# rhuangr/MARL-Maze

Measured on AMD Instinct MI355X. Metric: env-steps/sec (2-agent 10x10 maze) + PPO updates/sec, higher is better.
Workload: dtype f32; 1 GPU; PPO rollout+GAE+update over 65536 parallel 10x10 2-agent mazes per GPU (configs[2], the north-star workload: 65,536 parallel 10x10 mazes per GPU); mazes_per_gpu=65536, maze=10x10 (layout 19x19), horizon=16, global_batch=1048575, minibatch=209715, minibatch_steps_per_iter=25, parallelism=dp1, rollout=stream launches, gemm=x2, parity_mode=True

## Files before the change

include/marlmaze.h:

```cpp
#ifndef MARLMAZE_H
#define MARLMAZE_H

#include <stdint.h>

#ifdef __cplusplus
extern "C" {
#endif

#define MM_OBS_DIM 65
#define MM_MASK_DIM 6
#define MM_RNG_WORDS 625
#define MM_MAX_SIDE 41
#define MM_MAZES_PER_BLOCK 32

#define MM_E_ARG (-1)
#define MM_E_SIZE (-2)

#define MM_ST_GEN_FAIL 1u
#define MM_ST_BAD_MOVE 2u

typedef struct {
    int8_t x, y, dir, flags;
    int8_t lmx, lmy, olsx, olsy;
    int8_t minx, maxx, miny, maxy;
// ... 247 lines not shown
#define MM_PAR_HIST0 16
#define MM_PAR_HIST_BINS 16
int mm_par_init(uint64_t* totals, int32_t* counted, int n, void* stream);
int mm_par_accum(const uint8_t* done, const float* reward, const int32_t* ep_stats, const int32_t* par, int n,
                 int quota, int32_t* counted, uint64_t* totals, void* stream);

#define MM_ELOG_WORDS 16
#define MM_ELOG_LEN 0
#define MM_ELOG_SHORTEST 1
#define MM_ELOG_SOLVED 2
#define MM_ELOG_PAR 3
#define MM_ELOG_T_KEY 4
#define MM_ELOG_FETCHER 5
#define MM_ELOG_T_KNOW0 6
#define MM_ELOG_T_KNOW1 7
#define MM_ELOG_T_READY 8
#define MM_ELOG_CELLS0 9
#define MM_ELOG_CELLS1 10
#define MM_ELOG_CELLS_BOTH 11
#define MM_ELOG_OPEN 12
#define MM_ELOG_MARKS0 13
#define MM_ELOG_MARKS1 14
#define MM_ELOG_STAYS 15
long mm_elog_state_words(int layout_stride);
int mm_elog_init(int32_t* log, int32_t* counted, int32_t* state, int n, int quota, long state_words, void* stream);
int mm_elog_start(const mm_env_t* env, const uint8_t* select, int32_t* state, long state_words, void* stream);
int mm_elog_step(const mm_env_t* env, const int8_t* actions, const uint8_t* done, const float* reward,
                 const int32_t* ep_stats, const int32_t* par, int quota, int32_t* counted, int32_t* state,
                 long state_words, int32_t* log, void* stream);

int mm_critic_value(const float* x, int ldx, int K0, int M, int H0, int H1, const float* w0, const float* b0,
                    const float* w1, const float* b1, const float* w2, const float* b2, float* v, void* stream);

int mm_actor_front_ws_len(void);
int mm_actor_front_prep(const float* const* wproj, const float* const* bproj, const float* wq, const float* wk,
                        const float* wv, float* ws, void* stream);
int mm_actor_front_fwd(const float* ws, const float* x, int ldx, int B, int parity, float* h, void* stream);

#define MM_FRONT_FWD_ROW1 0
#define MM_FRONT_FWD_ROW2 1
#define MM_FRONT_FWD_MFMA 2
int mm_actor_front_fwd_ex(const float* ws, const float* x, int ldx, int B, int parity, float* h, int algo,
                          void* stream);

int mm_actor_front_grad_len(void);
int mm_actor_front_partial_len(void);
int mm_actor_front_bwd(const float* ws, const float* x, int ldx, int B, int parity, const float* dh, float* partial,
                       int grid, float* red, float* grad, void* stream);
#define MM_FRONT_BWD_MFMA 0
#define MM_FRONT_BWD_VALU 1
int mm_actor_front_bwd_ex(const float* ws, const float* x, int ldx, int B, int parity, const float* dh,
                          float* partial, int grid, float* red, float* grad, int algo, void* stream);
int mm_actor_front_bwd_grid(int B, int algo);
int mm_actor_front_bwd_to(const float* ws, const float* x, int ldx, int B, int parity, const float* dh,
                          float* partial, int grid, float* red, float* const* wproj_grad, float* const* bproj_grad,
                          float* wq_grad, float* wk_grad, float* wv_grad, int algo, void* stream);

#ifdef __cplusplus
}
#endif
#endif
```

marl-maze_amd/csrc/x3mlp.hip:

```cpp
#include <hip/hip_runtime.h>
#include <stdint.h>
#include <stdlib.h>

#include <algorithm>
#include <type_traits>

#include "marlmaze.h"
#include "policy_device.h"

namespace mm {
namespace x3 {

typedef __attribute__((ext_vector_type(8))) short bf16x8;
typedef __attribute__((ext_vector_type(4))) float f32x4;
typedef __attribute__((ext_vector_type(8))) _Float16 f16x8;

enum { P_X3 = MM_PREC_X3, P_F16 = MM_PREC_F16, P_X2 = MM_PREC_X2 };
template <int P>
struct Prec {
    static constexpr int kPlanes = P == P_X3 ? 3 : P == P_X2 ? 2 : 1;
    static constexpr int kBlk = 512 * kPlanes;
    static constexpr bool kScaled = P != P_X3;
};
constexpr float kX2Lo = 2048.f;
// ... 2369 lines not shown
                if (odd) bres_step<P, CT, RT, VW>(acc, accx, rawA, rawB, as, ks, K, kq, ctb, c0, ctn, ascale, sF, lane);
                if (half) {
#pragma unroll
                    for (int r = 0; r < RT; r++) bres_frag16<P, VW>(odd ? rawB[r] : rawA[r], ascale, a4[r]);
                }
            }
            if (half) {
                const uint2* bp = reinterpret_cast<const uint2*>(sT) + (size_t)(c0 * np) * 64 + lane;
#pragma unroll
                for (int c = 0; c < CT; c++) {
                    if (c < ctn) {
                        uint2 bb[3];
#pragma unroll
                        for (int q = 0; q < np; q++) bb[q] = bp[(c * np + q) * 64];
#pragma unroll
                        for (int r = 0; r < RT; r++) acc[r][c] = mma16<P>(a4[r], bb, acc[r][c], accx[r][c]);
                    }
                }
            }
#pragma unroll
            for (int r = 0; r < RT; r++)
#pragma unroll
                for (int c = 0; c < CT; c++) acc[r][c] = x2_combine<P>(acc[r][c], accx[r][c]);
#pragma unroll
            for (int r = 0; r < RT; r++)
                bres_epilogue<P, CT, EM>(acc[r], RT * u + r, t0 + c0, ctn, M, N, ep, crs, srs, sbias + 16 * c0, lane);
        }
        X3_STAMP(1 + t, 2, __builtin_amdgcn_s_memtime());
    }
    X3_STAMP(0, 3, __builtin_amdgcn_s_memtime());
    X3_STAMP(0, 5, __builtin_amdgcn_s_memrealtime());
}

}
}

using namespace mm::x3;

#ifdef X3_STAMPS
extern "C" int mm_x3_stamps_read(unsigned long long* out, long n) {
    const long cap = (long)(sizeof(g_x3_stamps) / sizeof(g_x3_stamps[0]));
    return hipMemcpyFromSymbol(out, HIP_SYMBOL(g_x3_stamps), (n < cap ? n : cap) * sizeof(unsigned long long), 0,
                               hipMemcpyDeviceToHost) == hipSuccess ? 0 : -1;
}
extern "C" int mm_trunk_stamps_read(unsigned long long* out, long n) {
    const long cap = (long)(sizeof(g_tr_stamps) / sizeof(g_tr_stamps[0]));
    return hipMemcpyFromSymbol(out, HIP_SYMBOL(g_tr_stamps), (n < cap ? n : cap) * sizeof(unsigned long long), 0,
                               hipMemcpyDeviceToHost) == hipSuccess ? 0 : -1;
}
extern "C" int mm_x3_stamps_clear() {
    static unsigned long long zero[256 * 16 * kWaves * 8];
    return hipMemcpyToSymbol(HIP_SYMBOL(g_x3_stamps), zero, sizeof(zero), 0, hipMemcpyHostToDevice) == hipSuccess
               ? 0 : -1;
}
#endif

extern "C" long mm_x3_tp_len(int R, int C) { return (long)(rup(R, kRowPad) / 16) * (rup(C, 32) / 32) * kBlk; }

extern "C" long mm_gemm_tp_len(int prec, int R, int C) {
    if (prec != MM_PREC_X3 && prec != MM_PREC_F16 && prec != MM_PREC_X2) return MM_E_ARG;
    return mm_x3_tp_len(R, C) / 3 * (prec == MM_PREC_X3 ? 3 : prec == MM_PREC_X2 ? 2 : 1);
}

extern "C" long mm_x3_mbits_len(int M) { return (long)(rup(M, kRowPad) / 16) * 64 * kMaskWords; }

extern "C" int mm_gemm_tp_pack(int prec, const float* X, int R, int C, int ld, int trans, uint16_t* tp,
// ... 826 lines not shown
}

extern "C" int mm_gemm_wgrad_partials_h(int prec, int flags, const float* dy, int lddy, float dscale, const void* x,
                                        int ldx, int M, int N, int K, float cscale, float* ws, void* stream) {
    if (M <= 0) return MM_E_ARG;
    return gemm_wgrad(prec, dy, lddy, dscale, static_cast<const float*>(x), ldx, M, N, K, cscale, ws, nullptr, stream,
                      flags);
}

extern "C" int mm_gemm_a16_ok(int M, int N, int K, int lda, int ldc) {
    BresPlan pl;
    int cfg = C_NARROW;
    return bres_enabled() && bres_plan(MM_PREC_F16, M, N, K, lda, ldc, true, pl, cfg) ? 1 : 0;
}

extern "C" int mm_gemm_x2p_ok(int M, int N, int K) {
    if (M <= 0 || N <= 0 || K <= 0 || N > 16 * kWgMaxT || (N & 3) || (K & 3)) return 0;
    if ((size_t)(M + 16) * std::max(N, K) * 4 >= ((size_t)1 << 31)) return 0;
    return wg_x2p_shape(wg_plan(MM_PREC_X2, M, N, K)) ? 1 : 0;
}

extern "C" int mm_gemm_wgrad_slices(int prec, int M, int N, int K) {
    if (M <= 0 || N <= 0 || K <= 0 || (prec != MM_PREC_X3 && prec != MM_PREC_F16 && prec != MM_PREC_X2))
        return MM_E_ARG;
    const WgPlan p = wg_plan(prec, M, N, K);
    return p.TPW ? p.nslices : MM_E_ARG;
}

extern "C" int mm_gemm_wgrad_partials(int prec, const float* dy, int lddy, float dscale, const float* x, int ldx, int M,
                                      int N, int K, float cscale, float* ws, void* stream) {
    if (M <= 0) return MM_E_ARG;
    return gemm_wgrad(prec, dy, lddy, dscale, x, ldx, M, N, K, cscale, ws, nullptr, stream);
}
```

marl-maze_amd/marlmaze/PPO.py:

```python
import math
import os
import random
import warnings

import numpy as np
import torch

from . import _lib, networks, ops, rollout, update, x3
from .dist import DP
from .networks import Actor, Critic

MODEL_PATH = "PPO.pth"
CRITIC_STREAM = os.environ.get("MARLMAZE_CRITIC_STREAM", "on")
CRITIC_STREAM_MAX_SAMPLES = int(os.environ.get("MARLMAZE_CRITIC_STREAM_MAX", "65536"))


def _ppo_loss_fwd(heads, mk, a8, old_logp, adv, clip):
    L = _lib.lib()
    M = old_logp.shape[0]
    old_logp, adv = old_logp.contiguous(), adv.contiguous()
    coef = torch.empty(M, dtype=torch.float32, device=heads.device)
    part = torch.empty(L.mm_ppo_loss_partials(M), dtype=torch.float32, device=heads.device)
    _lib.check(L.mm_ppo_loss(_lib.ptr(heads), _lib.ptr(mk), _lib.ptr(a8), _lib.ptr(old_logp), _lib.ptr(adv), M,
                             float(clip), _lib.ptr(coef), _lib.ptr(part), _lib.stream_ptr()), "mm_ppo_loss")
# ... 138 lines not shown
        return self._replay.graph

    def _carry_over(self):
        rollout.carry_over(self)

    def get_batch(self):
        return rollout.episode_batch(self) if self.episode_batches else rollout.horizon_batch(self)

    def policy_logp(self, obs, act, masks):
        M = obs.shape[0]
        ml, kl = self.actor(obs.reshape(2 * M, 65))
        mk = masks.reshape(2 * M, 6).bool()
        a = act.reshape(2 * M, 2)
        ml = ml.masked_fill(~mk[:, 0:5], float("-inf"))
        lp = torch.log_softmax(ml, dim=-1).gather(1, a[:, 0:1].long()).squeeze(1)
        kl = kl.squeeze(1).masked_fill(~mk[:, 5], float("-inf"))
        p = torch.sigmoid(kl)
        p = torch.where(a[:, 1] != 0, p, 1 - p)
        lp = (lp + torch.log(p)).view(M, 2)
        return lp[:, 0] + lp[:, 1]

    def minibatch_grads(self, obs, act, old_logp, adv, rtg, masks, out=None):
        if not obs.is_cuda:
            return self._minibatch_grads_host(obs, act, old_logp, adv, rtg, masks)
        M = obs.shape[0]
        a8 = (act if act.dtype == torch.int8 else act.to(torch.int8)).contiguous()
        mk = _u8(masks)
        if out is None:
            out = torch.empty(2, dtype=torch.float32, device=obs.device)
        beside = CRITIC_STREAM == "on" or (CRITIC_STREAM == "auto" and M <= CRITIC_STREAM_MAX_SAMPLES)
        with x3.cached_packs():
            x3.pack_many(self.critic.pack_specs() + self.actor.pack_specs())
            with _lib.on_side(_lib.side_stream("critic", obs.device) if beside else None) as critic_side:
                V, csaved = self.critic.train_forward(obs.reshape(M, -1))
                mse_part, dv = update.mse_loss(V, rtg)
                with x3.deferred():
                    self.critic.train_backward(csaved, dv)
            heads, asaved = self.actor.train_forward(obs.reshape(2 * M, 65))
            coef, ppo_part = _ppo_loss_fwd(heads, mk, a8, old_logp, adv, self.clip)
            dz = _ppo_loss_bwd(heads, mk, a8, coef, self._one)
            with x3.deferred():
                self.actor.train_backward(asaved, dz)
            critic_side.join(mse_part)
            update.losses_final(ppo_part, mse_part, M, out)
        return out[0], out[1]

    def _minibatch_grads_host(self, obs, act, old_logp, adv, rtg, masks):
        V = self.critic(obs).view(-1)
        cur = self.policy_logp(obs, act, masks)
        ratio = torch.exp(cur - old_logp)
        s1 = ratio * adv
        s2 = torch.clamp(ratio, 1 - self.clip, 1 + self.clip) * adv
        actor_loss = -torch.mean(torch.min(s1, s2))
        critic_loss = torch.nn.functional.mse_loss(V, rtg)
        self.actor_optim.zero_grad(set_to_none=True)
        self.critic_optim.zero_grad(set_to_none=True)
        (actor_loss + critic_loss).backward()
        return actor_loss.detach(), critic_loss.detach()

    def minibatch_step(self, obs, act, old_logp, adv, rtg, masks, out=None):
        if self.flat is None:
            return self._minibatch_step_host(obs, act, old_logp, adv, rtg, masks)
        if out is None:
            out = torch.empty(4, dtype=torch.float32, device=obs.device)
        self.minibatch_grads(obs, act, old_logp, adv, rtg, masks, out=out[0:2])
        scale = 1.0
        if self.dp.active:
            self.dp.allreduce_sum(self.flat.grad)
            scale = 1.0 / self.dp.world
        update.clip_adam([self.actor_optim, self.critic_optim], self.max_grad, norms=out[2:4], grad_scale=scale)
# ... 212 lines not shown
```

marl-maze_amd/marlmaze/_lib.py:

```python
import ctypes
import os

import torch

PKG_ROOT = os.path.dirname(os.path.dirname(os.path.abspath(__file__)))
LIB_PATH = os.environ.get("MARLMAZE_LIB") or os.path.join(PKG_ROOT, "libmarlmaze.so")

OBS_DIM = 65
MASK_DIM = 6
RNG_WORDS = 625
MAX_SIDE = 41
MAZES_PER_BLOCK = 32

ST_GEN_FAIL = 1
ST_BAD_MOVE = 2

GAE_AUTO, GAE_COLUMN, GAE_WALK, GAE_SCAN = 0, 1, 2, 3

ACT_SAMPLE, ACT_GREEDY = 0, 1
ACT_MODES = {"sample": ACT_SAMPLE, "greedy": ACT_GREEDY}

EVAL_WORDS = 32
EV_EPISODES, EV_SOLVED, EV_TIMEOUTS, EV_SUM_LEN, EV_SUM_LEN_SOLVED, EV_SUM_SHORT_SOLVED = 0, 1, 2, 3, 4, 5
EV_MIN_LEN_SOLVED, EV_MAX_LEN_SOLVED, EV_SUM_RATIO_Q16, EV_BAD_SHORT = 6, 7, 8, 9
# ... 5 lines not shown
PAR_HIST0, PAR_HIST_BINS = 16, 16

ELOG_WORDS = 16
ELOG_LEN, ELOG_SHORTEST, ELOG_SOLVED, ELOG_PAR, ELOG_T_KEY, ELOG_FETCHER, ELOG_T_KNOW0, ELOG_T_KNOW1 = range(8)
ELOG_T_READY, ELOG_CELLS0, ELOG_CELLS1, ELOG_CELLS_BOTH, ELOG_OPEN, ELOG_MARKS0, ELOG_MARKS1, ELOG_STAYS = range(8, 16)
ELOG_FIELDS = ("LEN", "SHORTEST", "SOLVED", "PAR", "T_KEY", "FETCHER", "T_KNOW0", "T_KNOW1", "T_READY", "CELLS0",
               "CELLS1", "CELLS_BOTH", "OPEN", "MARKS0", "MARKS1", "STAYS")

AF_KNOWS_END = 1
AF_SEES_END = 2
AF_OTHER_KNOWS = 4
AF_HAS_KEY = 8
AF_SEES_KEY = 16
AF_TEAM_KEY = 32
AF_HAS_MARK = 64

EXPORTS = ("mm_version", "mm_env_desc_size", "mm_layout_stride", "mm_env_seed", "mm_env_reset",
           "mm_env_step", "mm_env_step_timed", "mm_env_reset_done", "mm_env_pregen", "mm_gae", "mm_gae_ex", "mm_sample", "mm_head_sample", "mm_head_sample_ex", "mm_heads_fwd",
           "mm_actor_front_ws_len", "mm_actor_front_prep", "mm_actor_front_fwd", "mm_actor_front_fwd_ex",
           "mm_actor_front_grad_len", "mm_actor_front_partial_len", "mm_actor_front_bwd", "mm_actor_front_bwd_ex",
           "mm_actor_front_bwd_to", "mm_actor_front_bwd_grid",
           "mm_x3_tp_len", "mm_x3_tp_pack", "mm_x3_nt", "mm_x3_nt_f32a", "mm_x3_mbits_len",
           "mm_x3_heads_bwd", "mm_ppo_loss_partials", "mm_ppo_loss", "mm_ppo_loss_bwd",
           "mm_gemm_tp_len", "mm_gemm_tp_pack", "mm_gemm_nt", "mm_gemm_nt_algo", "mm_gemm_wgrad_algo", "mm_gemm_wgrad_ws_len",
           "mm_gemm_wgrad", "mm_colsum", "mm_mse_loss_partials", "mm_mse_loss", "mm_losses_final",
           "mm_clip_adam_ws_len", "mm_clip_adam", "mm_gemm_tp_pack_multi", "mm_gemm_wgrad_slices",
           "mm_gemm_wgrad_partials", "mm_colsum_multi_ws_len", "mm_colsum_multi", "mm_wsum_multi", "mm_critic_value",
           "mm_gemm_range_flag", "mm_gemm_nt_h", "mm_gemm_a16_ok", "mm_gemm_wgrad_h", "mm_gemm_wgrad_partials_h",
           "mm_heads_fwd_h16", "mm_x3_heads_bwd_h16", "mm_trunk3_ok", "mm_trunk3",
           "mm_trunk3_head_sample_ok", "mm_trunk3_head_sample", "mm_actor_front_fwd_h16",
           "mm_actor_front_fwd_h16_ex", "mm_head_act", "mm_act", "mm_eval_init", "mm_eval_accum",
           "mm_env_dist", "mm_env_par", "mm_par_init", "mm_par_accum",
           "mm_elog_state_words", "mm_elog_init", "mm_elog_start", "mm_elog_step",
           "mm_gemm_x2p_ok", "mm_x3_heads_bwd_x2p")
VERSION = 308

PREC_X3, PREC_F16, PREC_X2 = 0, 1, 2
FRONT_BWD = {"mfma": 0, "valu": 1}
FRONT_FWD = {"row1": 0, "row2": 1, "mfma": 2}
GEMM_ALGO = {"auto": 0, "stream": 1}
GEMM_A_F16, GEMM_C_F16, GEMM_B_F16 = 1, 2, 4
GEMM_A_X2P, GEMM_C_X2P, GEMM_B_X2P = 8, 16, 32


class EnvDesc(ctypes.Structure):
    _fields_ = [
        ("n", ctypes.c_int32), ("size_w", ctypes.c_int32), ("size_h", ctypes.c_int32),
        ("max_timestep", ctypes.c_int32), ("difficulty", ctypes.c_int32),
        ("rand_start", ctypes.c_int32), ("rand_sizes", ctypes.c_int32),
        ("rand_lo", ctypes.c_int32), ("rand_hi", ctypes.c_int32),
        ("layout_stride", ctypes.c_int32),
        ("layout", ctypes.c_void_p), ("agents", ctypes.c_void_p), ("mazes", ctypes.c_void_p),
        ("rng", ctypes.c_void_p), ("work", ctypes.c_void_p),
        ("next_layout", ctypes.c_void_p), ("next_mazes", ctypes.c_void_p), ("next_rng", ctypes.c_void_p),
        ("gen_state", ctypes.c_void_p),
    ]


class AdamSeg(ctypes.Structure):
    _fields_ = [
        ("param", ctypes.c_void_p), ("grad", ctypes.c_void_p), ("exp_avg", ctypes.c_void_p),
        ("exp_avg_sq", ctypes.c_void_p), ("n", ctypes.c_long), ("max_norm", ctypes.c_float),
        ("step_size", ctypes.c_float), ("bc2_sqrt", ctypes.c_float), ("grad_scale", ctypes.c_float),
    ]


class PackSeg(ctypes.Structure):
# ... 140 lines not shown
        L.mm_gemm_tp_pack.restype = i32
        L.mm_gemm_nt.argtypes = [i32, P, i32, f32, P, i32, i32, i32, P, i32, P, P, P, f32, P, i32, P]
        L.mm_gemm_nt.restype = i32
        L.mm_gemm_nt_algo.argtypes = [i32]
        L.mm_gemm_nt_algo.restype = i32
        L.mm_gemm_wgrad_algo.argtypes = [i32]
        L.mm_gemm_wgrad_algo.restype = i32
        L.mm_gemm_wgrad_ws_len.argtypes = [i32, i32, i32]
        L.mm_gemm_wgrad_ws_len.restype = ctypes.c_long
        L.mm_gemm_wgrad.argtypes = [i32, P, i32, f32, P, i32, i32, i32, i32, f32, P, P, P]
        L.mm_gemm_wgrad.restype = i32
        L.mm_gemm_tp_pack_multi.argtypes = [i32, ctypes.POINTER(PackSeg), i32, P]
        L.mm_gemm_tp_pack_multi.restype = i32
        L.mm_gemm_wgrad_slices.argtypes = [i32, i32, i32, i32]
        L.mm_gemm_wgrad_slices.restype = i32
        L.mm_gemm_wgrad_partials.argtypes = [i32, P, i32, f32, P, i32, i32, i32, i32, f32, P, P]
        L.mm_gemm_wgrad_partials.restype = i32
        L.mm_gemm_range_flag.argtypes = [P, i32, P]
        L.mm_gemm_range_flag.restype = i32
        for name, args in (("mm_gemm_nt_h", [i32, i32, P, i32, f32, P, i32, i32, i32, P, i32, P, P, P, f32, f32, P, i32,
                                             P]),
                           ("mm_x3_heads_bwd_h16", [P, i32, P, P, i32, i32, P, P, f32, P]),
                           ("mm_gemm_a16_ok", [i32, i32, i32, i32, i32]),
                           ("mm_gemm_wgrad_h", [i32, i32, P, i32, f32, P, i32, i32, i32, i32, f32, P, P, P]),
                           ("mm_gemm_wgrad_partials_h", [i32, i32, P, i32, f32, P, i32, i32, i32, i32, f32, P, P]),
                           ("mm_heads_fwd_h16", [P, i32, i32, P, P, i32, P, P]),
                           ("mm_trunk3_ok", [i32, i32, i32, i32, i32, i32, i32]),
                           ("mm_trunk3", [i32, P, i32, i32, i32, P, P, i32, P, P, i32, P, P, i32, P, i32, P]),
                           ("mm_trunk3_head_sample_ok", [i32, i32, i32, i32, i32, i32, i32]),
                           ("mm_actor_front_fwd_h16", [P, P, i32, i32, i32, P, P]),
                           ("mm_actor_front_fwd_h16_ex", [P, P, i32, i32, i32, P, i32, P]),
                           ("mm_gemm_x2p_ok", [i32, i32, i32]),
                           ("mm_x3_heads_bwd_x2p", [P, i32, P, P, i32, i32, P, P, f32, P]),
                           ("mm_trunk3_head_sample", [i32, P, i32, i32, i32, P, P, i32, P, P, i32, P, P, i32, P, P, P,
                                                      u64, u64, P, P, P, P, P, P, i32, P])):
            if hasattr(L, name):
                getattr(L, name).argtypes = args
                getattr(L, name).restype = i32
        L.mm_colsum_multi_ws_len.argtypes = [ctypes.POINTER(ColsumSeg), i32]
        L.mm_colsum_multi_ws_len.restype = ctypes.c_long
        L.mm_colsum_multi.argtypes = [ctypes.POINTER(ColsumSeg), i32, P, P]
        L.mm_colsum_multi.restype = i32
        L.mm_wsum_multi.argtypes = [ctypes.POINTER(WsumSeg), i32, P]
        L.mm_wsum_multi.restype = i32
        L.mm_x3_mbits_len.argtypes = [i32]
        L.mm_x3_mbits_len.restype = ctypes.c_long
        L.mm_x3_nt_f32a.restype = i32
        L.mm_actor_front_ws_len.restype = i32
        L.mm_actor_front_prep.argtypes = [ctypes.POINTER(P), ctypes.POINTER(P), P, P, P, P, P]
        L.mm_actor_front_prep.restype = i32
        L.mm_actor_front_fwd.argtypes = [P, P, i32, i32, i32, P, P]
        L.mm_actor_front_fwd.restype = i32
        L.mm_actor_front_fwd_ex.argtypes = [P, P, i32, i32, i32, P, i32, P]
        L.mm_actor_front_fwd_ex.restype = i32
        L.mm_actor_front_grad_len.restype = i32
        L.mm_actor_front_partial_len.restype = i32
        L.mm_actor_front_bwd_grid.argtypes = [i32, i32]
        L.mm_actor_front_bwd_grid.restype = i32
        L.mm_actor_front_bwd.argtypes = [P, P, i32, i32, i32, P, P, i32, P, P, P]
        L.mm_actor_front_bwd.restype = i32
        L.mm_actor_front_bwd_ex.argtypes = [P, P, i32, i32, i32, P, P, i32, P, P, i32, P]
        L.mm_actor_front_bwd_ex.restype = i32
        if L.mm_version() // 100 != VERSION // 100 or L.mm_env_desc_size() != ctypes.sizeof(EnvDesc):
            raise MMError(f"{LIB_PATH}: ABI {L.mm_version()} / mm_env_t of {L.mm_env_desc_size()} bytes, "
                          f"this binding expects {VERSION} / {ctypes.sizeof(EnvDesc)}: rebuild the library")
        _LIB = L
# ... 53 lines not shown
```

marl-maze_amd/marlmaze/networks.py:

```python
import ctypes
import math
import os

import numpy as np
import torch
import torch.nn as nn
import torch.nn.functional as F

FEATURE_DIMS = [4, 4, 4, 4, 4, 4, 4, 4, 4, 4, 4, 4, 2, 2, 1, 4, 1, 1, 1, 1, 1, 1, 2]
FEATURE_AMOUNT = len(FEATURE_DIMS)
OBS_SPACE = int(np.sum(FEATURE_DIMS))
EMBEDDING_DIM = 20
KQ_DIM = 10
_SQRT_KQ = float(np.sqrt(KQ_DIM))


class Projection(nn.Module):

    def __init__(self, parity_mode=True):
        super().__init__()
        self.layers = nn.ModuleList([nn.Linear(d, EMBEDDING_DIM) for d in FEATURE_DIMS])
        self.parity_mode = parity_mode
        starts = np.zeros(FEATURE_AMOUNT, np.int64) if parity_mode else np.cumsum([0] + FEATURE_DIMS[:-1])
        self.register_buffer("_starts", torch.as_tensor(starts), persistent=False)
# ... 110 lines not shown
def _engine_ok(x, widths):
    return x.is_cuda and x.dim() == 2 and x.stride(1) == 1 and all(n <= _MAX_WIDTH for n in widths)


def _warn_torch_path(what):
    if what not in _WARNED:
        _WARNED.add(what)
        import warnings

        warnings.warn(f"marlmaze: {what} is outside the hand-written GEMM engine's shapes; it runs as plain "
                      "torch ops", RuntimeWarning, stacklevel=3)


def _grad_scale(M, prec):
    return float(2.0 ** int(math.floor(math.log2(max(int(M), 1))))) if prec in ("f16", "x2") else 1.0


def _wgrad(dy, x, prec, out=None, nk=None):
    from . import x3

    s = _grad_scale(dy.shape[0], prec)
    if x3.is_planes(dy):
        return x3.wgrad(dy, x, prec=prec, dscale=1.0, cscale=1.0 / s, out=out, nk=nk)
    if dy.dtype == torch.float16:
        return x3.wgrad(dy.contiguous(), x, prec=prec, dscale=1.0, cscale=1.0 / s, out=out)
    return x3.wgrad(dy.contiguous(), x, prec=prec, dscale=s, out=out)


F16_ACT = os.environ.get("MARLMAZE_F16_ACT", "1") != "0"
F16_H0 = os.environ.get("MARLMAZE_F16_H0", "1") != "0"


X2_PLANES = os.environ.get("MARLMAZE_X2_PLANES", "1") != "0"


class _SavedPlanes(torch.Tensor):

    _STORAGE = ("as_subclass",)

    @staticmethod
    def __new__(cls, p):
        return torch.Tensor._make_subclass(cls, p)

    def planes(self):
        return self.as_subclass(torch.Tensor)

    def values(self):
        p = self.planes()
        return (p[:, :, 0, :].float() + p[:, :, 1, :].float() * (1.0 / 2048.0)).reshape(p.shape[0], -1)

    @classmethod
    def __torch_function__(cls, func, types, args=(), kwargs=None):
        kwargs = kwargs or {}
        if getattr(func, "__name__", "") in cls._STORAGE:
            with torch._C.DisableTorchFunctionSubclass():
                return func(*args, **kwargs)
        from torch.utils._pytree import tree_map

        def val(a):
            return a.values() if isinstance(a, _SavedPlanes) else a

        return func(*tree_map(val, args), **tree_map(val, kwargs))


def _x2p(prec, M, shapes):
    from . import x3
# ... 470 lines not shown
            if torch.is_grad_enabled() and any(p.requires_grad for p in params):
                return _EngineCritic.apply(self.gemm_prec, x, *params)
            with torch.no_grad():
                return _critic_fwd(x, params, self.gemm_prec, False)[0]
        act = self.activation()
        for lin in self.layers[:-1]:
            x = act(F.linear(x, lin.weight, lin.bias))
        return F.linear(x, self.layers[-1].weight, self.layers[-1].bias)

    @torch.no_grad()
    def value_into(self, x, out):
        from . import _lib

        x = x.reshape(-1, self.agent_amount * OBS_SPACE)
        if not self._engine(x):
            out.copy_(self(x).reshape(out.shape))
            return out
        w0, b0, w1, b1, w2, b2 = self._params()
        if (len(self.layers) == 3 and w0.shape[0] == 64 and w0.shape[1] == x.shape[1] and w1.shape == (64, 64)
                and w2.shape == (1, 64) and x.shape[1] <= 132 and out.is_contiguous()):
            _lib.check(_lib.lib().mm_critic_value(_lib.ptr(x), x.stride(0), x.shape[1], x.shape[0], 64, 64,
                                                   *(_lib.ptr(t) for t in (w0, b0, w1, b1, w2, b2)), _lib.ptr(out),
                                                   _lib.stream_ptr()), "mm_critic_value")
            return out
        _critic_fwd(x, self._params(), self.gemm_prec, False, out=out.view(-1, 1))
        return out

    def train_forward(self, x):
        x = x.reshape(-1, self.agent_amount * OBS_SPACE).contiguous()
        assert x.is_cuda and self._engine(x)
        v, hs, bits = _critic_fwd(x, self._params(), self.gemm_prec, True)
        return v, (hs, bits)

    def pack_specs(self):
        ws = [lin.weight for lin in self.layers]
        return [(w, False, self.gemm_prec) for w in ws] + [(w, True, self.gemm_prec) for w in ws[1:-1]]

    def train_backward(self, saved, dv):
        hs, bits = saved
        params = self._params()
        _critic_bwd(hs, bits, params, dv.reshape(-1, 1).contiguous(), self.gemm_prec,
                    outs=[_grad_of(p) for p in params])
```

marl-maze_amd/marlmaze/update.py:

```python
import math

import torch

from . import _lib, x3

_ALIGN = 4


class FlatParams:

    def __init__(self, segments, adjacent=()):
        glued = {id(p): i for i, grp in enumerate(adjacent) for p in grp[1:]}
        dev = segments[0][0].device
        self.segs = []
        self.offsets = {}
        off = 0
        for params in segments:
            start = off
            for p in params:
                if id(p) not in glued:
                    off = (off + _ALIGN - 1) // _ALIGN * _ALIGN
                self.offsets[id(p)] = off
                off += p.numel()
            off = (off + _ALIGN - 1) // _ALIGN * _ALIGN
# ... 115 lines not shown

def clip_adam(opts, max_norm, norms=None, grad_scale=1.0):
    L = _lib.lib()
    f = opts[0].flat
    g0 = opts[0].param_groups[0]
    for o in opts:
        g = o.param_groups[0]
        if tuple(g["betas"]) != tuple(g0["betas"]) or g["eps"] != g0["eps"] or o.flat is not f:
            raise ValueError("clip_adam steps optimizers with the same betas / eps over one FlatParams")
    segs = (_lib.AdamSeg * len(opts))(*[o.segment(max_norm, grad_scale) for o in opts])
    ws = _workspace(f.data.device, L.mm_clip_adam_ws_len(len(opts)))
    b1, b2 = g0["betas"]
    _lib.check(L.mm_clip_adam(segs, len(opts), float(b1), float(b2), float(g0["eps"]), _lib.ptr(ws),
                              _lib.ptr(norms), _lib.stream_ptr()), "mm_clip_adam")
    for o in opts:
        o.t += 1
    x3.invalidate_packs()


_WS = {}


def _workspace(dev, n):
    key = (str(dev), int(n))
    if key not in _WS:
        _WS[key] = torch.empty(int(n), dtype=torch.float32, device=dev)
    return _WS[key]


def mse_loss(v, rtg, dv=None):
    L = _lib.lib()
    M = v.numel()
    v, rtg = v.reshape(M).contiguous(), rtg.reshape(M).contiguous()
    if dv is None:
        dv = torch.empty(M, dtype=torch.float32, device=v.device)
    part = torch.empty(L.mm_mse_loss_partials(M), dtype=torch.float32, device=v.device)
    _lib.check(L.mm_mse_loss(_lib.ptr(v), _lib.ptr(rtg), M, _lib.ptr(dv), _lib.ptr(part), _lib.stream_ptr()),
               "mm_mse_loss")
    return part, dv


def losses_final(ppo_part, mse_part, M, out):
    _lib.check(_lib.lib().mm_losses_final(_lib.ptr(ppo_part), ppo_part.numel(), _lib.ptr(mse_part),
                                          mse_part.numel(), int(M), _lib.ptr(out), _lib.stream_ptr()),
               "mm_losses_final")
    return out
```

Before: 7.484 million env-steps/s.

## Fuse critic forward, MSE gradient and activation backward into one persistent kernel

Adds a persistent HIP kernel that runs, per 16-row tile, the three-layer critic MLP forward, the value loss gradient, and the backward through the ReLU layers. Weights stay resident in LDS and the work uses f16 MFMA with split-precision planes. It writes h0, h1, dy1 and dy0 plus per-tile column sums for the later weight-gradient GEMMs, replacing several separate forward, MSE and backward launches and their intermediate round trips. The MSE partial sums are still computed by the existing kernel. Weight gradients are still done by separate wgrad calls, so the kernel mainly removes launch overhead and intermediate reads, and it adds a constrained shape path that must stay numerically equivalent.

```diff
diff --git a/include/marlmaze.h b/include/marlmaze.h
--- a/include/marlmaze.h
+++ b/include/marlmaze.h
@@ -303,6 +303,12 @@
 int mm_critic_value(const float* x, int ldx, int K0, int M, int H0, int H1, const float* w0, const float* b0,
                     const float* w1, const float* b1, const float* w2, const float* b2, float* v, void* stream);
 
+int mm_critic_update_ok(int M, int K0, int ldx);
+int mm_critic_update(const float* x, int ldx, int K0, int M, const float* rtg, const uint16_t* w0_tp, const float* b0,
+                     const uint16_t* w1_tp, const uint16_t* w1t_tp, const float* b1, const uint16_t* w2_tp,
+                     const float* w2, const float* b2, float* v, float* dv, float* h0, float* h1, float* dy1,
+                     float* dy0, float* cs1, float* cs0, void* stream);
+
 int mm_actor_front_ws_len(void);
 int mm_actor_front_prep(const float* const* wproj, const float* const* bproj, const float* wq, const float* wk,
                         const float* wv, float* ws, void* stream);
diff --git a/marl-maze_amd/csrc/x3mlp.hip b/marl-maze_amd/csrc/x3mlp.hip
--- a/marl-maze_amd/csrc/x3mlp.hip
+++ b/marl-maze_amd/csrc/x3mlp.hip
@@ -2425,6 +2425,281 @@
     X3_STAMP(0, 5, __builtin_amdgcn_s_memrealtime());
 }
 
+constexpr int kCuWaves = 8;
+constexpr int kCuScr = 68;
+constexpr int kCuW0 = 0;
+constexpr int kCuT0 = kCuW0 + 32768;
+constexpr int kCuW1 = kCuT0 + 4096;
+constexpr int kCuW1T = kCuW1 + 16384;
+constexpr int kCuW2 = kCuW1T + 16384;
+constexpr int kCuScrOff = kCuW2 + 4096;
+constexpr int kCuLds = kCuScrOff + kCuWaves * 16 * kCuScr * 4;
+static_assert(kCuLds <= 160 * 1024, "k_critic_update's LDS");
+
+struct CuArgs {
+    const float* x;
+    int ldx, K0, M;
+    const float* rtg;
+    const uint16_t *w0, *w1, *w1t, *w2;
+    const float *b0, *b1, *w2f, *b2;
+    float gscale, norm;
+    float *v, *dv;
+    float *h0, *h1, *dy1, *dy0;
+    float *cs1, *cs0;
+};
+
+__device__ __forceinline__ void cu_wave_sync() {
+    __builtin_amdgcn_fence(__ATOMIC_RELEASE, "wavefront");
+    __builtin_amdgcn_wave_barrier();
+    __builtin_amdgcn_fence(__ATOMIC_ACQUIRE, "wavefront");
+}
+
+__device__ __forceinline__ void cu_put(float* scr, const f32x4 (&t)[4], int lane) {
+    float* p = scr + 4 * (lane >> 4) * kCuScr + (lane & 15);
+#pragma unroll
+    for (int c = 0; c < 4; c++)
+#pragma unroll
+        for (int g = 0; g < 4; g++) p[g * kCuScr + 16 * c] = t[c][g];
+}
+
+template <int NT>
+__device__ __forceinline__ void cu_mma(const bf16x8 (&a)[3], const bf16x8 (&b)[NT][2], f32x4 (&acc)[NT],
+                                       f32x4 (&accx)[NT]) {
+#define MM_H8(x) __builtin_bit_cast(f16x8, x)
+#pragma unroll
+    for (int c = 0; c < NT; c++) accx[c] = __builtin_amdgcn_mfma_f32_16x16x32_f16(MM_H8(a[1]), MM_H8(b[c][0]), accx[c], 0, 0, 0);
+#pragma unroll
+    for (int c = 0; c < NT; c++) accx[c] = __builtin_amdgcn_mfma_f32_16x16x32_f16(MM_H8(a[0]), MM_H8(b[c][1]), accx[c], 0, 0, 0);
+#pragma unroll
+    for (int c = 0; c < NT; c++) acc[c] = __builtin_amdgcn_mfma_f32_16x16x32_f16(MM_H8(a[0]), MM_H8(b[c][0]), acc[c], 0, 0, 0);
+#undef MM_H8
+}
+template <int NT>
+__device__ __forceinline__ void cu_mma16(const uint2 (&a)[2], const uint2 (&b)[NT][2], f32x4 (&acc)[NT],
+                                         f32x4 (&accx)[NT]) {
+    typedef __attribute__((ext_vector_type(4))) _Float16 h4;
+#define MM_H4(x) __builtin_bit_cast(h4, x)
+#pragma unroll
+    for (int c = 0; c < NT; c++) accx[c] = __builtin_amdgcn_mfma_f32_16x16x16f16(MM_H4(a[1]), MM_H4(b[c][0]), accx[c], 0, 0, 0);
+#pragma unroll
+    for (int c = 0; c < NT; c++) accx[c] = __builtin_amdgcn_mfma_f32_16x16x16f16(MM_H4(a[0]), MM_H4(b[c][1]), accx[c], 0, 0, 0);
+#pragma unroll
+    for (int c = 0; c < NT; c++) acc[c] = __builtin_amdgcn_mfma_f32_16x16x16f16(MM_H4(a[0]), MM_H4(b[c][0]), acc[c], 0, 0, 0);
+#undef MM_H4
+}
+
+template <int NT>
+__device__ __forceinline__ void cu_layer64(const float* scr, float s, const unsigned char* sB, int lane,
+                                           f32x4 (&acc)[NT]) {
+    f32x4 accx[NT];
+#pragma unroll
+    for (int c = 0; c < NT; c++) acc[c] = accx[c] = f32x4{0.f, 0.f, 0.f, 0.f};
+    const float* ar = scr + (lane & 15) * kCuScr + 4 * (lane >> 4);
+#pragma unroll
+    for (int ks = 0; ks < 2; ks++) {
+        float4 raw[2];
+        raw[0] = *reinterpret_cast<const float4*>(ar + 32 * ks);
+        raw[1] = *reinterpret_cast<const float4*>(ar + 32 * ks + 16);
+        bf16x8 a[3];
+        a[2] = bf16x8{0, 0, 0, 0, 0, 0, 0, 0};
+        bres_frag<P_X2, 4>(raw, s, a);
+        const bf16x8* bp = reinterpret_cast<const bf16x8*>(sB) + (ks * NT * 2) * 64 + lane;
+        bf16x8 bb[NT][2];
+#pragma unroll
+        for (int c = 0; c < NT; c++) bb[c][0] = bp[(c * 2) * 64], bb[c][1] = bp[(c * 2 + 1) * 64];
+        cu_mma<NT>(a, bb, acc, accx);
+    }
+#pragma unroll
+    for (int c = 0; c < NT; c++) acc[c] = x2_combine<P_X2>(acc[c], accx[c]);
+}
+
+__global__ __launch_bounds__(64 * kCuWaves) void k_critic_update(CuArgs ca) {
+    extern __shared__ __attribute__((aligned(16))) uint16_t smem[];
+    unsigned char* sm = reinterpret_cast<unsigned char*>(smem);
+    const int lane = threadIdx.x & 63;
+    const int wave = __builtin_amdgcn_readfirstlane(threadIdx.x >> 6);
+    const int K0 = ca.K0, M = ca.M, ldx = ca.ldx;
+    constexpr int nks0 = 5, nfull = 4;
+
+    for (int i = threadIdx.x; i < nfull * 8 * 64; i += 64 * kCuWaves) {
+        const int p = i >> 6, q = p & 1, c = (p >> 1) & 3, ks = p >> 3;
+        reinterpret_cast<uint4*>(sm + kCuW0)[i] =
+            reinterpret_cast<const uint4*>(ca.w0 + ((size_t)c * nks0 + ks) * 1024 + q * 512)[i & 63];
+    }
+    for (int i = threadIdx.x; i < 8 * 64; i += 64 * kCuWaves) {
+        const int p = i >> 6, q = p & 1, c = p >> 1;
+        reinterpret_cast<uint2*>(sm + kCuT0)[i] =
+            reinterpret_cast<const uint2*>(ca.w0 + ((size_t)c * nks0 + nfull) * 1024 + q * 512)[2 * (i & 63)];
+    }
+    for (int i = threadIdx.x; i < 16 * 64; i += 64 * kCuWaves) {
+        const int p = i >> 6, q = p & 1, c = (p >> 1) & 3, ks = p >> 3;
+        const size_t o = ((size_t)c * 2 + ks) * 1024 + q * 512;
+        reinterpret_cast<uint4*>(sm + kCuW1)[i] = reinterpret_cast<const uint4*>(ca.w1 + o)[i & 63];
+        reinterpret_cast<uint4*>(sm + kCuW1T)[i] = reinterpret_cast<const uint4*>(ca.w1t + o)[i & 63];
+    }
+    for (int i = threadIdx.x; i < 4 * 64; i += 64 * kCuWaves) {
+        const int p = i >> 6, q = p & 1, ks = p >> 1;
+        reinterpret_cast<uint4*>(sm + kCuW2)[i] =
+            reinterpret_cast<const uint4*>(ca.w2 + (size_t)ks * 1024 + q * 512)[i & 63];
+    }
+    __syncthreads();
+
+    const int cl = lane & 15, rq = 4 * (lane >> 4), kq = 4 * (lane >> 4);
+    float b0r[4], b1r[4], w2r[4];
+#pragma unroll
+    for (int c = 0; c < 4; c++) b0r[c] = ca.b0[16 * c + cl], b1r[c] = ca.b1[16 * c + cl], w2r[c] = ca.w2f[16 * c + cl];
+    const float b2 = ca.b2[0], gs = ca.gscale, gsi = 1.f / ca.gscale, norm = ca.norm;
+    float* scr = reinterpret_cast<float*>(sm + kCuScrOff) + wave * 16 * kCuScr;
+    const __amdgpu_buffer_rsrc_t xrs =
+        __builtin_amdgcn_make_buffer_rsrc((void*)ca.x, (short)0, (int)((size_t)M * ldx * 4), 0x00020000);
+    const int obytes = (int)((size_t)M * 64 * 4);
+    const __amdgpu_buffer_rsrc_t rh0 = __builtin_amdgcn_make_buffer_rsrc((void*)ca.h0, (short)0, obytes, 0x00020000);
+    const __amdgpu_buffer_rsrc_t rh1 = __builtin_amdgcn_make_buffer_rsrc((void*)ca.h1, (short)0, obytes, 0x00020000);
+    const __amdgpu_buffer_rsrc_t ry1 = __builtin_amdgcn_make_buffer_rsrc((void*)ca.dy1, (short)0, obytes, 0x00020000);
+    const __amdgpu_buffer_rsrc_t ry0 = __builtin_amdgcn_make_buffer_rsrc((void*)ca.dy0, (short)0, obytes, 0x00020000);
+    uint32_t rm = 0u;
+
+    const int ntiles = (M + 15) / 16, stride = kCuWaves * (int)gridDim.x;
+    float4 raw[5][1][2];
+    {
+        BresA as;
+        as.rsrc = xrs;
+        as.roff[0] = as.roff[1] =
+            4u * ((uint32_t)min(16 * (kCuWaves * (int)blockIdx.x + wave) + cl, M - 1) * (uint32_t)ldx + (uint32_t)kq);
+#pragma unroll
+        for (int ks = 0; ks < 5; ks++) bres_load<1, 2>(as, ks, K0, kq, raw[ks]);
+    }
+    for (int rt = kCuWaves * (int)blockIdx.x + wave; rt < ntiles; rt += stride) {
+        bf16x8 af[4][3];
+        uint2 at[3];
+        at[2] = make_uint2(0u, 0u);
+#pragma unroll
+        for (int ks = 0; ks < 4; ks++) {
+            af[ks][2] = bf16x8{0, 0, 0, 0, 0, 0, 0, 0};
+            bres_frag<P_X2, 2>(raw[ks][0], 1.f, af[ks]);
+        }
+        bres_frag16<P_X2, 2>(raw[nfull][0], 1.f, at);
+        float rtgv[4];
+#pragma unroll
+        for (int g = 0; g < 4; g++) {
+            const int row = 16 * rt + rq + g;
+            rtgv[g] = (cl == 0 && row < M) ? ca.rtg[row] : 0.f;
+        }
+        {
+            BresA as;
+            as.rsrc = xrs;
+            as.roff[0] = as.roff[1] = 4u * ((uint32_t)min(16 * (rt + stride) + cl, M - 1) * (uint32_t)ldx + (uint32_t)kq);
+#pragma unroll
+            for (int ks = 0; ks < 5; ks++) bres_load<1, 2>(as, ks, K0, kq, raw[ks]);
+        }
+        uint32_t voff[4];
+#pragma unroll
+        for (int g = 0; g < 4; g++) voff[g] = 4u * ((uint32_t)(16 * rt + rq + g) * 64u + (uint32_t)cl);
+
+        f32x4 h0[4];
+        {
+            f32x4 accx[4];
+#pragma unroll
+            for (int c = 0; c < 4; c++) h0[c] = accx[c] = f32x4{0.f, 0.f, 0.f, 0.f};
+#pragma unroll
+            for (int ks = 0; ks < nfull; ks++) {
+                const bf16x8* bp = reinterpret_cast<const bf16x8*>(sm + kCuW0) + (ks * 8) * 64 + lane;
+                bf16x8 bb[4][2];
+#pragma unroll
+                for (int c = 0; c < 4; c++) bb[c][0] = bp[(c * 2) * 64], bb[c][1] = bp[(c * 2 + 1) * 64];
+                cu_mma<4>(af[ks], bb, h0, accx);
+            }
+            {
+                const uint2* bp = reinterpret_cast<const uint2*>(sm + kCuT0) + lane;
+                uint2 bb[4][2];
+#pragma unroll
+                for (int c = 0; c < 4; c++) bb[c][0] = bp[(c * 2) * 64], bb[c][1] = bp[(c * 2 + 1) * 64];
+                const uint2 a2[2] = {at[0], at[1]};
+                cu_mma16<4>(a2, bb, h0, accx);
+            }
+#pragma unroll
+            for (int c = 0; c < 4; c++) {
+                h0[c] = x2_combine<P_X2>(h0[c], accx[c]);
+                range_acc<P_X2>(rm, h0[c]);
+#pragma unroll
+                for (int g = 0; g < 4; g++) {
+                    h0[c][g] = fmaxf(h0[c][g] + b0r[c], 0.f);
+                    __builtin_amdgcn_raw_buffer_store_b32(__float_as_uint(h0[c][g]), rh0, voff[g], 64 * c, 0);
+                }
+            }
+        }
+        cu_put(scr, h0, lane);
+        cu_wave_sync();
+
+        f32x4 h1[4];
+        cu_layer64<4>(scr, 1.f, sm + kCuW1, lane, h1);
+#pragma unroll
+        for (int c = 0; c < 4; c++) {
+            range_acc<P_X2>(rm, h1[c]);
+#pragma unroll
+            for (int g = 0; g < 4; g++) {
+                h1[c][g] = fmaxf(h1[c][g] + b1r[c], 0.f);
+                __builtin_amdgcn_raw_buffer_store_b32(__float_as_uint(h1[c][g]), rh1, voff[g], 64 * c, 0);
+            }
+        }
+        cu_wave_sync();
+        cu_put(scr, h1, lane);
+        cu_wave_sync();
+        f32x4 vv[1];
+        cu_layer64<1>(scr, 1.f, sm + kCuW2, lane, vv);
+        range_acc<P_X2>(rm, vv[0]);
+        float dvb[4];
+#pragma unroll
+        for (int g = 0; g < 4; g++) {
+            const int row = 16 * rt + rq + g;
+            float dv = 0.f;
+            if (cl == 0 && row < M) {
+                const float v = vv[0][g] + b2;
+                ca.v[row] = v;
+                dv = (v - rtgv[g]) * norm;
+                ca.dv[row] = dv;
+            }
+            dvb[g] = __shfl(dv, lane & 48);
+        }
+
+        const bool tile_ok = lane < 16;
+        f32x4 dy[4];
+#pragma unroll
+        for (int c = 0; c < 4; c++) {
+            float cs = 0.f;
+#pragma unroll
+            for (int g = 0; g < 4; g++) {
+                dy[c][g] = h1[c][g] > 0.f ? fmaf(dvb[g], w2r[c], 0.f) : 0.f;
+                if (16 * rt + rq + g < M) cs += dy[c][g];
+                __builtin_amdgcn_raw_buffer_store_b32(__float_as_uint(dy[c][g]), ry1, voff[g], 64 * c, 0);
+            }
+            cs += __shfl_xor(cs, 16);
+            cs += __shfl_xor(cs, 32);
+            if (tile_ok) ca.cs1[(size_t)rt * 64 + 16 * c + cl] = cs;
+        }
+        cu_wave_sync();
+        cu_put(scr, dy, lane);
+        cu_wave_sync();
+        cu_layer64<4>(scr, gs, sm + kCuW1T, lane, dy);
+#pragma unroll
+        for (int c = 0; c < 4; c++) {
+            range_acc<P_X2>(rm, dy[c]);
+            float cs = 0.f;
+#pragma unroll
+            for (int g = 0; g < 4; g++) {
+                dy[c][g] = (h0[c][g] > 0.f && 16 * rt + rq + g < M) ? dy[c][g] * gsi : 0.f;
+                cs += dy[c][g];
+                __builtin_amdgcn_raw_buffer_store_b32(__float_as_uint(dy[c][g]), ry0, voff[g], 64 * c, 0);
+            }
+            cs += __shfl_xor(cs, 16);
+            cs += __shfl_xor(cs, 32);
+            if (tile_ok) ca.cs0[(size_t)rt * 64 + 16 * c + cl] = cs;
+        }
+        cu_wave_sync();
+    }
+    range_note_wave<P_X2>(__builtin_amdgcn_ballot_w64(rm >= 0x7F800000u));
+}
+
 }
 }
 
@@ -3317,3 +3592,43 @@
     if (M <= 0) return MM_E_ARG;
     return gemm_wgrad(prec, dy, lddy, dscale, x, ldx, M, N, K, cscale, ws, nullptr, stream);
 }
+
+extern "C" int mm_critic_update_ok(int M, int K0, int ldx) {
+    if (M <= 0 || K0 <= 128 || K0 > 132 || (K0 & 1) || (ldx & 1) || ldx < K0) return 0;
+    const size_t wmax = std::max(ldx, 64);
+    if ((size_t)(M + 320) * wmax * 4 >= ((size_t)1 << 31)) return 0;
+    if (!bres_enabled()) return 0;
+    BresPlan pl;
+    int cfg = C_PAIR;
+    return bres_plan(MM_PREC_X2, M, 64, K0, ldx, 64, true, pl, cfg) && bres_plan(MM_PREC_X2, M, 64, 64, 64, 64, true, pl, cfg) &&
+                   bres_plan(MM_PREC_X2, M, 1, 64, 64, 1, false, pl, cfg)
+               ? 1
+               : 0;
+}
+
+extern "C" int mm_critic_update(const float* x, int ldx, int K0, int M, const float* rtg, const uint16_t* w0_tp,
+                                const float* b0, const uint16_t* w1_tp, const uint16_t* w1t_tp, const float* b1,
+                                const uint16_t* w2_tp, const float* w2, const float* b2, float* v, float* dv,
+                                float* h0, float* h1, float* dy1, float* dy0, float* cs1, float* cs0,
+                                void* stream) {
+    if (!x || !rtg || !w0_tp || !b0 || !w1_tp || !w1t_tp || !b1 || !w2_tp || !w2 || !b2 || !v || !dv || !h0 ||
+        !h1 || !dy1 || !dy0 || !cs1 || !cs0)
+        return MM_E_ARG;
+    if (((uintptr_t)x & 7) || (((uintptr_t)w0_tp | (uintptr_t)w1_tp | (uintptr_t)w1t_tp | (uintptr_t)w2_tp) & 15))
+        return MM_E_ARG;
+    if (mm_critic_update_ok(M, K0, ldx) != 1) return MM_E_ARG;
+    static bool attr = false;
+    if (!attr) {
+        if (hipFuncSetAttribute((const void*)k_critic_update, hipFuncAttributeMaxDynamicSharedMemorySize, kCuLds) !=
+            hipSuccess)
+            return MM_E_ARG;
+        attr = true;
+    }
+    const int G = std::min(persistent_grid(), ((M + 15) / 16 + kCuWaves - 1) / kCuWaves);
+    int e2 = 0;
+    const float gscale = ldexpf(1.f, (frexpf((float)M, &e2), e2 - 1));
+    CuArgs ca{x, ldx, K0, M, rtg, w0_tp, w1_tp, w1t_tp, w2_tp, b0, b1, w2, b2, gscale, (float)(2.0 / (double)M),
+              v, dv, h0, h1, dy1, dy0, cs1, cs0};
+    hipLaunchKernelGGL(k_critic_update, dim3(G), dim3(64 * kCuWaves), kCuLds, (hipStream_t)stream, ca);
+    return (int)hipGetLastError();
+}
diff --git a/marl-maze_amd/marlmaze/PPO.py b/marl-maze_amd/marlmaze/PPO.py
--- a/marl-maze_amd/marlmaze/PPO.py
+++ b/marl-maze_amd/marlmaze/PPO.py
@@ -194,10 +194,14 @@
         with x3.cached_packs():
             x3.pack_many(self.critic.pack_specs() + self.actor.pack_specs())
             with _lib.on_side(_lib.side_stream("critic", obs.device) if beside else None) as critic_side:
-                V, csaved = self.critic.train_forward(obs.reshape(M, -1))
-                mse_part, dv = update.mse_loss(V, rtg)
-                with x3.deferred():
-                    self.critic.train_backward(csaved, dv)
+                xc = obs.reshape(M, -1)
+                if self.critic.fused_update_ok(xc):
+                    _, mse_part = self.critic.train_update_fused(xc, rtg)
+                else:
+                    V, csaved = self.critic.train_forward(xc)
+                    mse_part, dv = update.mse_loss(V, rtg)
+                    with x3.deferred():
+                        self.critic.train_backward(csaved, dv)
             heads, asaved = self.actor.train_forward(obs.reshape(2 * M, 65))
             coef, ppo_part = _ppo_loss_fwd(heads, mk, a8, old_logp, adv, self.clip)
             dz = _ppo_loss_bwd(heads, mk, a8, coef, self._one)
diff --git a/marl-maze_amd/marlmaze/_lib.py b/marl-maze_amd/marlmaze/_lib.py
--- a/marl-maze_amd/marlmaze/_lib.py
+++ b/marl-maze_amd/marlmaze/_lib.py
@@ -61,7 +61,8 @@
            "mm_actor_front_fwd_h16_ex", "mm_head_act", "mm_act", "mm_eval_init", "mm_eval_accum",
            "mm_env_dist", "mm_env_par", "mm_par_init", "mm_par_accum",
            "mm_elog_state_words", "mm_elog_init", "mm_elog_start", "mm_elog_step",
-           "mm_gemm_x2p_ok", "mm_x3_heads_bwd_x2p")
+           "mm_gemm_x2p_ok", "mm_x3_heads_bwd_x2p",
+           "mm_critic_update_ok", "mm_critic_update")
 VERSION = 308
 
 PREC_X3, PREC_F16, PREC_X2 = 0, 1, 2
@@ -268,6 +269,8 @@
                            ("mm_actor_front_fwd_h16_ex", [P, P, i32, i32, i32, P, i32, P]),
                            ("mm_gemm_x2p_ok", [i32, i32, i32]),
                            ("mm_x3_heads_bwd_x2p", [P, i32, P, P, i32, i32, P, P, f32, P]),
+                           ("mm_critic_update_ok", [i32, i32, i32]),
+                           ("mm_critic_update", [P, i32, i32, i32] + [P] * 18),
                            ("mm_trunk3_head_sample", [i32, P, i32, i32, i32, P, P, i32, P, P, i32, P, P, i32, P, P, P,
                                                       u64, u64, P, P, P, P, P, P, i32, P])):
             if hasattr(L, name):
diff --git a/marl-maze_amd/marlmaze/networks.py b/marl-maze_amd/marlmaze/networks.py
--- a/marl-maze_amd/marlmaze/networks.py
+++ b/marl-maze_amd/marlmaze/networks.py
@@ -166,6 +166,8 @@
 
 
 X2_PLANES = os.environ.get("MARLMAZE_X2_PLANES", "1") != "0"
+
+CRITIC_FUSED = os.environ.get("MARLMAZE_CRITIC_FUSED", "1") != "0"
 
 
 class _SavedPlanes(torch.Tensor):
@@ -702,6 +704,50 @@
         v, hs, bits = _critic_fwd(x, self._params(), self.gemm_prec, True)
         return v, (hs, bits)
 
+    def fused_update_ok(self, x):
+        from . import _lib
+
+        if not (CRITIC_FUSED and self.gemm_prec == "x2" and x.is_cuda and x.dtype == torch.float32
+                and x.dim() == 2 and x.stride(1) == 1 and len(self.layers) == 3 and self.activation is nn.ReLU):
+            return False
+        w0, w1, w2 = (lin.weight for lin in self.layers)
+        if not (w0.shape == (64, x.shape[1]) and w1.shape == (64, 64) and w2.shape == (1, 64)):
+            return False
+        return _lib.lib().mm_critic_update_ok(x.shape[0], x.shape[1], x.stride(0)) == 1
+
+    def train_update_fused(self, x, rtg, grads=None):
+        from . import _lib, update, x3
+
+        assert self.fused_update_ok(x), "train_update_fused: see fused_update_ok"
+        L = _lib.lib()
+        M, K0 = x.shape
+        dev = x.device
+        params = self._params()
+        w0, b0, w1, b1, w2, b2 = params
+        o = grads if grads is not None else [_grad_of(p) for p in params]
+        rtg = rtg.reshape(M).contiguous()
+        assert rtg.dtype == torch.float32 and rtg.is_cuda
+        prec = self.gemm_prec
+        p0, p1, p1t, p2 = (x3.pack(w0, prec=prec), x3.pack(w1, prec=prec), x3.pack(w1, trans=True, prec=prec),
+                           x3.pack(w2, prec=prec))
+        v = torch.empty((M, 1), dtype=torch.float32, device=dev)
+        dv = torch.empty((M, 1), dtype=torch.float32, device=dev)
+        h0, h1, dy1, dy0 = (torch.empty((M, 64), dtype=torch.float32, device=dev) for _ in range(4))
+        cs1, cs0 = x3.colsum_buf(M, 64, dev), x3.colsum_buf(M, 64, dev)
+        _lib.check(L.mm_critic_update(_lib.ptr(x), x.stride(0), K0, M, _lib.ptr(rtg), p0.ptr(), _lib.ptr(b0), p1.ptr(),
+                                      p1t.ptr(), _lib.ptr(b1), p2.ptr(), _lib.ptr(w2), _lib.ptr(b2),
+                                      *(_lib.ptr(t) for t in (v, dv, h0, h1, dy1, dy0, cs1, cs0)),
+                                      _lib.stream_ptr()), "mm_critic_update")
+        part, _ = update.mse_loss(v, rtg, dv=False)
+        with x3.deferred():
+            _wgrad(dv, h1, prec, out=o[4])
+            x3.colsum(dv, out=o[5])
+            _wgrad(dy1, h0, prec, out=o[2], nk=tuple(w1.shape))
+            x3.colsum(cs1, out=o[3])
+            _wgrad(dy0, x.contiguous(), prec, out=o[0], nk=tuple(w0.shape))
+            x3.colsum(cs0, out=o[1])
+        return v, part
+
     def pack_specs(self):
         ws = [lin.weight for lin in self.layers]
         return [(w, False, self.gemm_prec) for w in ws] + [(w, True, self.gemm_prec) for w in ws[1:-1]]
diff --git a/marl-maze_amd/marlmaze/update.py b/marl-maze_amd/marlmaze/update.py
--- a/marl-maze_amd/marlmaze/update.py
+++ b/marl-maze_amd/marlmaze/update.py
@@ -171,7 +171,9 @@
     L = _lib.lib()
     M = v.numel()
     v, rtg = v.reshape(M).contiguous(), rtg.reshape(M).contiguous()
-    if dv is None:
+    if dv is False:
+        dv = None
+    elif dv is None:
         dv = torch.empty(M, dtype=torch.float32, device=v.device)
     part = torch.empty(L.mm_mse_loss_partials(M), dtype=torch.float32, device=v.device)
     _lib.check(L.mm_mse_loss(_lib.ptr(v), _lib.ptr(rtg), M, _lib.ptr(dv), _lib.ptr(part), _lib.stream_ptr()),
```

After: 7.578 million env-steps/s, median of 6. 1.3% higher.
